# nekStab/nekStab_next

Measured on AMD Instinct MI355X. Metric: Arnoldi-step GB/s (achieved HBM) + Ritz-value rel-err, N=1e8 m=128, higher is better.
Workload: dtype f64

## Files before the change

include/nekkrylov.h:

```cpp
#ifndef NEKKRYLOV_H
#define NEKKRYLOV_H

#include <stddef.h>
#include <stdint.h>

#ifdef __cplusplus
extern "C" {
#endif

#define NKV_ABI_VERSION 3

#define NKV_TILE 4096
#define NKV_MAX_COLS 1024
#define NKV_ROT_MAX_OUT 256

#define NKV_OK 0
#define NKV_EINVAL 1
#define NKV_EHIP 2
#define NKV_ENAN 3
#define NKV_ESHAPE 4
#define NKV_ECALLBACK 5
#define NKV_EBREAKDOWN 6

#define NKV_TIME 0x1u
// ... 38 lines not shown
                 unsigned flags, void* stream);
int nkv_normalize_dev(const nkv_layout* L, double* x, const double* nrm2_dev, double* beta_dev,
                      unsigned flags, void* stream);

int nkv_dot(const nkv_layout* L, const double* w, const double* a, const double* b, double* out_dev,
            void* ws, unsigned flags, void* stream);

int nkv_block_dot(const nkv_layout* L, const double* w, const double* Q, int j, const double* f,
                  double* h_dev, void* ws, unsigned flags, void* stream);
int nkv_block_update(const nkv_layout* L, const double* w, const double* Q, int j, const double* h_dev,
                     double* f, double* nrm2_dev, void* ws, unsigned flags, void* stream);
int nkv_block_update_dot(const nkv_layout* L, const double* w, const double* Q, int j, const double* h_dev,
                         double* f, double* hout_dev, void* ws, unsigned flags, void* stream);
int nkv_arnoldi_finish(const nkv_layout* L, const double* f, const double* nrm2_dev, double* q_out,
                       int j, const double* h1_dev, const double* h2_dev, double* hcol_dev,
                       unsigned flags, void* stream);

int nkv_combine(const nkv_layout* L, const double* Q, int k, const double* y_dev, double* out, unsigned flags,
                void* stream);
int nkv_normalize_store(const nkv_layout* L, const double* f, const double* nrm2_dev, double* q_next,
                        double* beta_dev, unsigned flags, void* stream);
int nkv_mgs2_step(const nkv_layout* L, const double* w, const double* Q, int j, double* f, double* q_out,
                  double* hcol_dev, void* ws, unsigned flags, void* stream);
int nkv_axpy_dot(const nkv_layout* L, const double* w, double* f, const double* alpha_dev, const double* qa,
                 const double* qb, double* out_dev, void* ws, unsigned flags, void* stream);

int nkv_block_dot2(const nkv_layout* L, const double* w, const double* Q, int j, const double* x,
                   const double* y, double* h_dev, void* ws, unsigned flags, void* stream);
int nkv_dcgs2_coef(int m, const double* hq_dev, const double* hw_dev, const double* nrm_prev_dev, double* H_dev,
                   int64_t ldh, double* coef_dev, void* ws, void* stream);
int nkv_dcgs2_update(const nkv_layout* L, const double* w, const double* Q, int m, const double* coef_dev,
                     double* qj, const double* win, double* fout, double* nrm2_dev, void* ws, unsigned flags,
                     void* stream);

int nkv_mgs_icwy_solve(int j, double* G, int64_t ldg, const double* grow, const double* b, double* x,
                       void* stream);

int nkv_gkl_coef(int side, int m, const double* hq_dev, const double* hw_dev, double* M_dev, int64_t ldm,
                 double* A_self, double* r_self, const double* A_other, const double* r_other, int64_t lda,
                 double* coef_dev, void* ws, void* stream);

typedef int (*nkv_matvec_fn)(void* user, const double* x, double* y, void* stream);
typedef int (*nkv_allreduce_fn)(void* user, double* buf, int n, void* stream);
size_t nkv_arnoldi_scratch_doubles(int m);
int nkv_arnoldi_dcgs2(const nkv_layout* L, const double* w, double* Q, int mstart, int mend, double* H_dev,
                      int64_t ldh, double* f, double* scratch_dev, void* ws, nkv_matvec_fn matvec, void* mv_user,
                      nkv_allreduce_fn allreduce, void* ar_user, unsigned flags, void* stream);

int nkv_gmres_dcgs2(const nkv_layout* L, const double* w, double* Q, int kmax, double beta, double tol2,
                    double* H_dev, int64_t ldh, double* f, double* scratch_dev, void* ws, nkv_matvec_fn matvec,
                    void* mv_user, nkv_allreduce_fn allreduce, void* ar_user, double* res_hist, int* k_out,
                    unsigned flags, void* stream);

int nkv_update_hessenberg(const nkv_layout* L, const double* w, const double* Q, int j, double* f, double* q_out,
                          double* hcol_dev, double* scratch_dev, void* ws, nkv_allreduce_fn allreduce, void* ar_user,
                          unsigned flags, void* stream);

int nkv_arnoldi_factorization(const nkv_layout* L, const double* w, double* Q, int mstart, int mend, double* H_dev,
                              int64_t ldh, double* f, double* scratch_dev, void* ws, nkv_matvec_fn matvec,
                              void* mv_user, nkv_allreduce_fn allreduce, void* ar_user, unsigned flags, void* stream);

int nkv_rotate(const nkv_layout* L, double* Q, int k, const double* V_dev, int ldv, void* stream);

int nkv_rotate_cols(const nkv_layout* L, double* Q, int k, const double* V_dev, int ldv, int n_out,
                    void* stream);

// ... 42 lines not shown
```

nekstab_next_amd/_lib.py:

```python
from __future__ import annotations

import ctypes
import os
from ctypes import CFUNCTYPE, POINTER, Structure, c_char_p, c_double, c_int, c_int32, c_int64, c_size_t, c_uint, c_uint64, c_void_p

import torch

_HERE = os.path.dirname(os.path.abspath(__file__))
LIB_PATH = os.path.join(_HERE, "libnekkrylov.so")

NKV_ABI_VERSION = 3
NKV_TILE = 4096
NKV_MAX_COLS = 1024
NKV_ROT_MAX_OUT = 256
NKV_OK, NKV_EINVAL, NKV_EHIP, NKV_ENAN, NKV_ESHAPE, NKV_ECALLBACK, NKV_EBREAKDOWN = 0, 1, 2, 3, 4, 5, 6
NKV_TIME = 0x1
NKV_ACCUMULATE = 0x2
NKV_OVERWRITE = 0x4
NKV_NORM2 = 0x8
NKV_TIME_DOT = 0x10
NKV_X_IS_LAST = 0x20
NKV_MGS2 = 0x40
NKV_MGS_ICWY = 0x100
NKV_MGS_LAGGED = 0x200
# ... 27 lines not shown
        ("n_wf", c_int32),
        ("rank0", c_int32),
    ]


_P = c_void_p
_L = POINTER(nkv_layout)
MATVEC_FN = CFUNCTYPE(c_int, c_void_p, c_void_p, c_void_p, c_void_p)
ALLREDUCE_FN = CFUNCTYPE(c_int, c_void_p, c_void_p, c_int, c_void_p)

_SIGNATURES = {
    "nkv_abi_version": (c_int, []),
    "nkv_layout_init": (c_int, [_L, c_int, c_int, c_int, c_int64, c_int64, c_int, c_int, c_int]),
    "nkv_last_error": (c_char_p, []),
    "nkv_device_info": (c_int, [POINTER(c_int), POINTER(c_int), POINTER(c_int64), c_char_p, c_int]),
    "nkv_workspace_bytes": (c_size_t, [_L, c_int]),
    "nkv_check_status": (c_int, [_P, _P]),
    "nkv_zero": (c_int, [_L, _P, c_uint, _P]),
    "nkv_copy": (c_int, [_L, _P, _P, c_uint, _P]),
    "nkv_scal": (c_int, [_L, _P, c_double, c_uint, _P]),
    "nkv_axpby": (c_int, [_L, _P, c_double, _P, c_double, c_uint, _P]),
    "nkv_sub3": (c_int, [_L, _P, _P, _P, c_uint, _P]),
    "nkv_axpy_dev": (c_int, [_L, _P, _P, c_double, _P, c_uint, _P]),
    "nkv_normalize_dev": (c_int, [_L, _P, _P, _P, c_uint, _P]),
    "nkv_dot": (c_int, [_L, _P, _P, _P, _P, _P, c_uint, _P]),
    "nkv_block_dot": (c_int, [_L, _P, _P, c_int, _P, _P, _P, c_uint, _P]),
    "nkv_block_update": (c_int, [_L, _P, _P, c_int, _P, _P, _P, _P, c_uint, _P]),
    "nkv_block_update_dot": (c_int, [_L, _P, _P, c_int, _P, _P, _P, _P, c_uint, _P]),
    "nkv_arnoldi_finish": (c_int, [_L, _P, _P, _P, c_int, _P, _P, _P, c_uint, _P]),
    "nkv_block_dot2": (c_int, [_L, _P, _P, c_int, _P, _P, _P, _P, c_uint, _P]),
    "nkv_dcgs2_coef": (c_int, [c_int, _P, _P, _P, _P, c_int64, _P, _P, _P]),
    "nkv_mgs_icwy_solve": (c_int, [c_int, _P, c_int64, _P, _P, _P, _P]),
    "nkv_dcgs2_update": (c_int, [_L, _P, _P, c_int, _P, _P, _P, _P, _P, _P, c_uint, _P]),
    "nkv_arnoldi_scratch_doubles": (c_size_t, [c_int]),
    "nkv_arnoldi_dcgs2": (c_int, [_L, _P, _P, c_int, c_int, _P, c_int64, _P, _P, _P, MATVEC_FN, _P, ALLREDUCE_FN, _P,
                                  c_uint, _P]),
    "nkv_update_hessenberg": (c_int, [_L, _P, _P, c_int, _P, _P, _P, _P, _P, ALLREDUCE_FN, _P, c_uint, _P]),
    "nkv_gmres_dcgs2": (c_int, [_L, _P, _P, c_int, c_double, c_double, _P, c_int64, _P, _P, _P, MATVEC_FN, _P,
                                ALLREDUCE_FN, _P, _P, _P, c_uint, _P]),
    "nkv_arnoldi_factorization": (c_int, [_L, _P, _P, c_int, c_int, _P, c_int64, _P, _P, _P, MATVEC_FN, _P,
                                          ALLREDUCE_FN, _P, c_uint, _P]),
    "nkv_combine": (c_int, [_L, _P, c_int, _P, _P, c_uint, _P]),
    "nkv_normalize_store": (c_int, [_L, _P, _P, _P, _P, c_uint, _P]),
    "nkv_mgs2_step": (c_int, [_L, _P, _P, c_int, _P, _P, _P, _P, c_uint, _P]),
    "nkv_axpy_dot": (c_int, [_L, _P, _P, _P, _P, _P, _P, _P, c_uint, _P]),
    "nkv_rotate": (c_int, [_L, _P, c_int, _P, c_int, _P]),
    "nkv_rotate_cols": (c_int, [_L, _P, c_int, _P, c_int, c_int, _P]),
    "nkv_op_diag": (c_int, [_L, _P, _P, _P, c_double, _P]),
    "nkv_op_rot2": (c_int, [_L, _P, _P, _P, _P, _P, c_int, _P]),
    "nkv_op_cdiag": (c_int, [_L, _P, _P, _P, _P, c_int, _P]),
    "nkv_fill_hash": (c_int, [_L, _P, c_uint64, c_int64, c_int64, _P]),
    "nkv_mth_rand_add": (c_int, [_L, c_int, c_int, c_int, c_int64, _P, _P, _P, c_double, c_double, c_double, _P, _P]),
    "nkv_group_average": (c_int, [c_int64, _P, _P, _P, _P]),
    "nkv_symmetric_seed": (c_int, [_L, _P, _P, c_double, _P, _P, _P, _P]),
    "nkv_wavemaker": (c_int, [_L, _P, _P, _P, _P, _P, c_int, _P]),
    "nkv_gradm1": (c_int, [_L, c_int, c_int, _P, _P, _P, _P, _P, c_int, c_int64, _P, c_int64, _P]),
    "nkv_bf_sensitivity": (c_int, [_L, _P, _P, _P, _P, _P, _P, c_int, _P]),
    "nkv_givens_column": (c_double, [c_int, _P, _P, _P, _P]),
    "nkv_lagged_coef": (c_int, [c_int, c_int, _P, _P, c_int64, _P, c_int64, _P]),
    "nkv_gkl_coef": (c_int, [c_int, c_int, _P, _P, _P, c_int64, _P, _P, _P, _P, c_int64, _P, _P, _P]),
    "nkv_sfd_step": (c_int, [_L, _P, _P, _P, _P, _P, _P, _P, _P, c_double, c_double, c_double, c_double, c_double,
                             c_int, _P, _P, c_uint, _P]),
    "nkv_tdf_step": (c_int, [_L, _P, _P, _P, _P, c_double, c_int, _P, _P, c_uint, _P]),
}

EXPORTED = tuple(_SIGNATURES)
# ... 52 lines not shown
```

nekstab_next_amd/arnoldi.py:

```python
from __future__ import annotations

import numpy as np
import torch

from . import _lib
from ._lib import NKV_NORM2, NKV_TIME, NKV_TIME_DOT, NKV_X_IS_LAST
from .operators import LinearOperator
from .vector import Basis, NekContext, NekVector


class HessenbergDev:

    def __init__(self, ctx: NekContext, k: int):
        self.ctx, self.k = ctx, k
        self.t = torch.zeros((k, k + 1), dtype=torch.float64, device=ctx.device)

    def col_ptr(self, c: int) -> int:
        return self.t[c].data_ptr()

    def download(self) -> np.ndarray:
        return np.asfortranarray(self.t.detach().cpu().numpy().T)

    def upload(self, H: np.ndarray) -> None:
        self.t.copy_(torch.as_tensor(np.ascontiguousarray(np.asarray(H, dtype=np.float64).T)).to(self.ctx.device))


def update_hessenberg_matrix(ctx: NekContext, Q: Basis, k: int, f: NekVector, Hd: HessenbergDev,
                             mode: str = "cgs2") -> None:
    j = int(k)
    if j + 1 > Q.k or j > ctx.max_cols:
        raise ValueError(f"step {j} exceeds basis size {Q.k} / max_cols {ctx.max_cols}")
    orthonormalize(ctx, Q, j, f, Q.col_ptr(j), Hd.col_ptr(j - 1), mode)


def orthonormalize(ctx: NekContext, Q: Basis, j: int, f: NekVector, out_ptr: int, hcol_ptr: int,
                   mode: str = "cgs2") -> None:
    w, ws, st = ctx.w.data_ptr(), ctx.ws.data_ptr(), ctx.stream
    if mode == "mgs2-icwy":
        raise ValueError("mode 'mgs2-icwy' keeps the basis's Gram matrix across steps: run it through "
                         "arnoldi_factorization (or use 'mgs2' for a single step)")
    if mode in ("cgs2-native", "mgs2-native"):
        scratch = _native_scratch(ctx, j)
        errors = []
        ar_c = _allreduce_callback(ctx, scratch, errors)
        flags = (NKV_TIME_DOT if ctx.time_in_dot else 0) | (_lib.NKV_MGS2 if mode == "mgs2-native" else 0)
        rc = ctx.lib.nkv_update_hessenberg(ctx._Lp, w, Q.ptr, int(j), f.ptr, out_ptr, hcol_ptr, scratch.data_ptr(), ws,
                                           ar_c, None, flags, st)
        if errors:
            raise errors[0]
        _lib.check(rc, "nkv_update_hessenberg")
        return
    if j == 0:
        tf = NKV_TIME if ctx.time_in_dot else 0
        nrm = ctx.scal[3:4]
        ctx.call("nkv_dot", w, f.ptr, f.ptr, nrm.data_ptr(), ws, tf, st)
        ctx.comm.allreduce_(nrm)
# ... 52 lines not shown
    w, ws, st = ctx.w.data_ptr(), ctx.ws.data_ptr(), ctx.stream
    lay, tm = ctx.layout, ctx.timer
    tf = NKV_TIME if ctx.time_in_dot else 0
    m = j - 1
    h = ctx.hd[: 2 * j]
    hp, cp = h.data_ptr(), ctx.coef.data_ptr()
    u = Q.col_ptr(m)
    if tm:
        tm.begin("block_dot2")
    ctx.call("nkv_block_dot2", w, Q.ptr, j, u, f.ptr, hp, ws, tf | NKV_X_IS_LAST, st)
    if tm:
        tm.end("block_dot2", 8.0 * ((j - 1) * lay.N_w + 2 * lay.N_w + lay.n_v))
    ctx.comm.allreduce_(h)
    nprev = None if first else (nrm2.data_ptr() if nrm2 is not None else hp + 8 * m)
    ctx.call_nl("nkv_dcgs2_coef", m, hp, hp + 8 * j, nprev, Hd.t.data_ptr(), Hd.k + 1, cp, ws, st)
    if tm:
        tm.begin("dcgs2_update")
    ctx.call("nkv_dcgs2_update", w, Q.ptr, m, cp, u, f.ptr, Q.col_ptr(j), None if nrm2 is None else nrm2.data_ptr(),
             ws, NKV_TIME | (NKV_TIME_DOT if tf else 0), st)
    if tm:
        tm.end("dcgs2_update", 8.0 * (m * lay.N + 4 * lay.N) + (0.0 if nrm2 is None else 8.0 * lay.n_v))
    if nrm2 is not None:
        ctx.comm.allreduce_(nrm2)


def _dcgs2_close(ctx: NekContext, Q: Basis, Hd: HessenbergDev, m: int) -> None:
    w, ws, st = ctx.w.data_ptr(), ctx.ws.data_ptr(), ctx.stream
    lay, tm = ctx.layout, ctx.timer
    tf = NKV_TIME if ctx.time_in_dot else 0
    h, coef = ctx.hd[: m + 1], ctx.coef
    u = Q.col_ptr(m)
    if tm:
        tm.begin("block_dot")
    ctx.call("nkv_block_dot", w, Q.ptr, m + 1, u, h.data_ptr(), ws, tf, st)
    if tm:
        tm.end("block_dot", 8.0 * ((m + 1) * lay.N_w + lay.N_w + lay.n_v))
    ctx.comm.allreduce_(h)
    ctx.call_nl("nkv_dcgs2_coef", m, h.data_ptr(), None, h.data_ptr() + 8 * m, Hd.t.data_ptr(), Hd.k + 1,
                coef.data_ptr(), ws, st)
    if tm:
        tm.begin("block_update")
    ctx.call("nkv_block_update", w, Q.ptr, m, h.data_ptr(), u, None, ws, NKV_TIME, st)
    if tm:
        tm.end("block_update", 8.0 * (m * lay.N + 2 * lay.N))
    ctx.call("nkv_normalize_dev", u, coef[2 * m + 3:].data_ptr(), None, 0, st)


def _icwy_gram(ctx: NekContext, Q: Basis, mstart: int) -> torch.Tensor:
    ldg = ctx.max_cols + 1
    G = getattr(ctx, "_icwy_G", None)
    if G is None:
        G = ctx._icwy_G = torch.zeros((ldg, ldg), dtype=torch.float64, device=ctx.device)
    w, ws, st = ctx.w.data_ptr(), ctx.ws.data_ptr(), ctx.stream
    tf = NKV_TIME if ctx.time_in_dot else 0
    for i in range(1, mstart - 1):
        ctx.call("nkv_block_dot", w, Q.ptr, i, Q.col_ptr(i), G[i].data_ptr(), ws, tf, st)
        ctx.comm.allreduce_(G[i, :i])
    return G


def _icwy_step(ctx: NekContext, Q: Basis, Hd: HessenbergDev, j: int, f: NekVector, G: torch.Tensor) -> None:
    w, ws, st = ctx.w.data_ptr(), ctx.ws.data_ptr(), ctx.stream
    lay, tm = ctx.layout, ctx.timer
    tf = NKV_TIME if ctx.time_in_dot else 0
    ldg = G.shape[1]
    h = ctx.hd[: 2 * j]
    hp, gp = h.data_ptr(), G.data_ptr()
    h1, h2, nrm = ctx.h1[:j], ctx.h2[:j], ctx.scal[3:4]
    if tm:
        tm.begin("block_dot2")
    ctx.call("nkv_block_dot2", w, Q.ptr, j, Q.col_ptr(j - 1), f.ptr, hp, ws, tf | NKV_X_IS_LAST, st)
    if tm:
        tm.end("block_dot2", 8.0 * ((j - 1) * lay.N_w + 2 * lay.N_w + lay.n_v))
    ctx.comm.allreduce_(h)
    ctx.call_nl("nkv_mgs_icwy_solve", j, gp, ldg, hp, hp + 8 * j, h1.data_ptr(), st)
    b_upd = 8.0 * (j * lay.N + 2 * lay.N)
    if tm:
        tm.begin("update_dot")
# ... 133 lines not shown
    scratch = _native_scratch(ctx, mend)
    base, ld8, fptr = Q.ptr, 8 * ctx.layout.ld, f.ptr
    apply = op.rmatvec if transpose else op.matvec
    errors = []

    def matvec(_user, x, y, _stream):
        try:
            c, r = divmod((x or 0) - base, ld8)
            if r or not 0 <= c < Q.k or y != fptr:
                raise ValueError(f"{entry} matvec callback: x={x}, y={y} are not a basis column and f")
            apply(Q[c], f)
            return 0
        except BaseException as e:
            errors.append(e)
            return 1

    mv_c = _lib.MATVEC_FN(matvec)
    ar_c = _allreduce_callback(ctx, scratch, errors)
    rc = getattr(lib, entry)(ctx._Lp, ctx.w.data_ptr(), Q.ptr, int(mstart), int(mend), Hd.t.data_ptr(), Hd.k + 1,
                             fptr, scratch.data_ptr(), ctx.ws.data_ptr(), mv_c, None, ar_c, None,
                             (NKV_TIME_DOT if ctx.time_in_dot else 0) | flags, ctx.stream)
    if errors:
        raise errors[0]
    _lib.check(rc, entry)


def arnoldi_factorization(ctx: NekContext, op: LinearOperator, Q: Basis, Hd: HessenbergDev, mstart: int,
                          mend: int, f: NekVector | None = None, mode: str = "cgs2", transpose: bool = False,
                          on_step=None) -> None:
    if mend < mstart:
        return
    if Q.k < mend + 1:
        raise ValueError("basis too small")
    if f is None:
        f = ctx.vector()
    if mode == "dcgs2-native":
        if on_step is None:
            if mend > ctx.max_cols or mend + 1 > Hd.k + 1:
                raise ValueError(f"step {mend} exceeds max_cols {ctx.max_cols} / H size {Hd.k}")
            _dcgs2_native(ctx, op, Q, Hd, mstart, mend, f, transpose)
            return
        mode = "dcgs2"
    if mode == "dcgs2" and on_step is not None:
        if mend > ctx.max_cols or mend + 1 > Hd.k + 1:
            raise ValueError(f"step {mend} exceeds max_cols {ctx.max_cols} / H size {Hd.k}")
        for mstep in range(mstart, mend + 1):
            (op.rmatvec if transpose else op.matvec)(Q[mstep - 1], f)
            _dcgs2_step(ctx, Q, Hd, mstep, f, first=(mstep == mstart))
            if mstep > mstart:
                on_step(mstep - 1)
        _dcgs2_close(ctx, Q, Hd, mend)
        on_step(mend)
        return
    if mode == "mgs2-lagged-native":
        if on_step is None:
            if mend > ctx.max_cols or mend + 1 > Hd.k + 1:
                raise ValueError(f"step {mend} exceeds max_cols {ctx.max_cols} / H size {Hd.k}")
            _dcgs2_native(ctx, op, Q, Hd, mstart, mend, f, transpose, entry="nkv_arnoldi_factorization",
                          flags=_lib.NKV_MGS_LAGGED)
            return
        mode = "mgs2-lagged"
    if mode == "mgs2-lagged":
        if mend > ctx.max_cols or mend + 1 > Hd.k + 1:
            raise ValueError(f"step {mend} exceeds max_cols {ctx.max_cols} / H size {Hd.k}")
        _lagged_factorization(ctx, op, Q, Hd, mstart, mend, f, transpose, on_step)
        return
# ... 26 lines not shown
            raise ValueError(f"step {mend} exceeds max_cols {ctx.max_cols} / H size {Hd.k}")
        for mstep in range(mstart, mend + 1):
            (op.rmatvec if transpose else op.matvec)(Q[mstep - 1], f)
            _dcgs2_step(ctx, Q, Hd, mstep, f, first=(mstep == mstart))
        _dcgs2_close(ctx, Q, Hd, mend)
        return
    if mode == "dcgs2":
        mode = "cgs2"
    for mstep in range(mstart, mend + 1):
        x = Q[mstep - 1]
        (op.rmatvec if transpose else op.matvec)(x, f)
        update_hessenberg_matrix(ctx, Q, mstep, f, Hd, mode)
        if on_step is not None:
            on_step(mstep)


class FactorizationGraph:

    def __init__(self, ctx: NekContext, op: LinearOperator, Q: Basis, Hd: HessenbergDev, f: NekVector,
                 mode: str = "cgs2"):
        self.ctx, self.op, self.Q, self.Hd, self.f, self.mode = ctx, op, Q, Hd, f, mode
        self.graphs = {}

    HOST_SYNC_MODES = ("mgs2-lagged", "mgs2-lagged-native")

    def usable(self) -> bool:
        return self.ctx.comm.world == 1 and self.mode not in self.HOST_SYNC_MODES

    def run(self, mstart: int, mend: int, transpose: bool = False) -> None:
        if mend < mstart:
            return
        key = (mstart, mend, transpose)
        Q = self.Q
        g = self.graphs.get(key)
        if g is None:
            timer, self.ctx.timer = self.ctx.timer, None
            g = torch.cuda.CUDAGraph()
            torch.cuda.synchronize(self.ctx.device)
            with torch.cuda.graph(g):
                arnoldi_factorization(self.ctx, self.op, Q, self.Hd, mstart, mend, f=self.f, mode=self.mode,
                                      transpose=transpose)
            self.ctx.timer = timer
            self.graphs[key] = g
        g.replay()
```

nekstab_next_amd/csrc/drivers.hip:

```cpp
#include "nkv_internal.h"

#include <vector>

extern "C" {

static size_t icwy_scratch_doubles(int m) { return (size_t)(4 * (m + 1) + 2) + (size_t)(m + 1) * (size_t)(m + 1); }
size_t nkv_arnoldi_scratch_doubles(int m) {
    const size_t base = (size_t)(2 * (m + 1) + 4 * m + 16), icwy = icwy_scratch_doubles(m);
    return base > icwy ? base : icwy;
}

static constexpr double kBreakdownTol = 1e-8;

static int check_breakdown(const double* H_dev, int64_t ldh, int c0, int c1, void* ws, void* stream) {
    if (c0 < 0) c0 = 0;
    if (c1 <= c0) return NKV_OK;
    hipStream_t st = S(stream);
    const size_t n = (size_t)ldh * (size_t)(c1 - c0);
    double* h = static_cast<double*>(malloc(n * sizeof(double)));
    if (!h) return fail(NKV_EINVAL, "breakdown check: host allocation of %zu doubles failed", n);
    int flag = 0;
    hipError_t e = hipMemcpyAsync(h, H_dev + (int64_t)c0 * ldh, n * sizeof(double), hipMemcpyDeviceToHost, st);
    if (e == hipSuccess) e = hipMemcpyAsync(&flag, nan_flag_of(ws), sizeof(int), hipMemcpyDeviceToHost, st);
    if (e == hipSuccess) e = hipStreamSynchronize(st);
// ... 20 lines not shown
        return fail(NKV_EBREAKDOWN, "breakdown at column %d: |H(c+1,c)|/||H(:,c)|| = %.3g (invariant subspace)",
                    bad, ratio);
    return NKV_OK;
}

int nkv_arnoldi_dcgs2(const nkv_layout* L, const double* w, double* Q, int mstart, int mend, double* H_dev,
                      int64_t ldh, double* f, double* scratch_dev, void* ws, nkv_matvec_fn matvec, void* mv_user,
                      nkv_allreduce_fn allreduce, void* ar_user, unsigned flags, void* stream) {
    CHECK(check_layout(L));
    CHECK(check_ptr(Q, "Q"));
    CHECK(check_ptr(f, "f"));
    if (!matvec) return fail(NKV_EINVAL, "matvec callback is NULL");
    if (!H_dev || !scratch_dev) return fail(NKV_EINVAL, "H/scratch is NULL");
    if (mstart < 1 || mend > NKV_MAX_COLS) return fail(NKV_EINVAL, "steps %d..%d outside 1..%d", mstart, mend, NKV_MAX_COLS);
    if (mend < mstart) return NKV_OK;
    if (ldh < mend + 1) return fail(NKV_EINVAL, "ldh=%lld < mend+1=%d", (long long)ldh, mend + 1);
    const unsigned tf = (flags & NKV_TIME_DOT) ? NKV_TIME : 0u;
    double* hd = scratch_dev;
    double* coef = scratch_dev + 2 * (mend + 1);
    auto col = [L, Q](int c) { return Q + (int64_t)c * L->ld; };
    for (int j = mstart; j <= mend; ++j) {
        const int m = j - 1;
        double* u = col(m);
        int rc = matvec(mv_user, u, f, stream);
        if (rc != 0) return fail(NKV_ECALLBACK, "matvec callback returned %d at step %d", rc, j);
        CHECK(nkv_block_dot2(L, w, Q, j, u, f, hd, ws, tf | NKV_X_IS_LAST, stream));
        if (allreduce && (rc = allreduce(ar_user, hd, 2 * j, stream)) != 0)
            return fail(NKV_ECALLBACK, "allreduce callback returned %d at step %d", rc, j);
        CHECK(nkv_dcgs2_coef(m, hd, hd + j, j == mstart ? nullptr : hd + m, H_dev, ldh, coef, ws, stream));
        CHECK(nkv_dcgs2_update(L, w, Q, m, coef, u, f, col(j), nullptr, ws, NKV_TIME, stream));
    }
    const int m = mend;
    double* u = col(m);
    CHECK(nkv_block_dot(L, w, Q, m + 1, u, hd, ws, tf, stream));
    if (allreduce) {
        const int rc = allreduce(ar_user, hd, m + 1, stream);
        if (rc != 0) return fail(NKV_ECALLBACK, "allreduce callback returned %d (closing step)", rc);
    }
    CHECK(nkv_dcgs2_coef(m, hd, nullptr, hd + m, H_dev, ldh, coef, ws, stream));
    CHECK(nkv_block_update(L, w, Q, m, hd, u, nullptr, ws, NKV_TIME, stream));
    CHECK(nkv_normalize_dev(L, u, coef + 2 * m + 3, nullptr, 0, stream));
    return (flags & NKV_CHECK_BREAKDOWN) ? check_breakdown(H_dev, ldh, mstart - 1, mend, ws, stream) : NKV_OK;
}

int nkv_gmres_dcgs2(const nkv_layout* L, const double* w, double* Q, int kmax, double beta, double tol2,
                    double* H_dev, int64_t ldh, double* f, double* scratch_dev, void* ws, nkv_matvec_fn matvec,
                    void* mv_user, nkv_allreduce_fn allreduce, void* ar_user, double* res_hist, int* k_out,
                    unsigned flags, void* stream) {
    CHECK(check_layout(L));
    CHECK(check_ptr(Q, "Q"));
    CHECK(check_ptr(f, "f"));
    CHECK(check_ptr(w, "w"));
    CHECK(check_ptr(ws, "ws"));
    if (!matvec) return fail(NKV_EINVAL, "matvec callback is NULL");
    if (!H_dev || !scratch_dev || !res_hist || !k_out) return fail(NKV_EINVAL, "H/scratch/res_hist/k_out is NULL");
    if (kmax < 1 || kmax + 1 > NKV_MAX_COLS) return fail(NKV_EINVAL, "kmax=%d outside 1..%d", kmax, NKV_MAX_COLS - 1);
    if (ldh < kmax + 1) return fail(NKV_EINVAL, "ldh=%lld < kmax+1=%d", (long long)ldh, kmax + 1);
    hipStream_t st = S(stream);
    const unsigned tf = (flags & NKV_TIME_DOT) ? NKV_TIME : 0u;
    double* hd = scratch_dev;
    double* coef = scratch_dev + 2 * (kmax + 1);
    double* nrm2 = scratch_dev + nkv_arnoldi_scratch_doubles(kmax) - 1;
    double* host = nullptr;
    if (hipHostMalloc(reinterpret_cast<void**>(&host), sizeof(double) * (size_t)(4 * (kmax + 2)),
                      hipHostMallocDefault) != hipSuccess || !host)
        return fail(NKV_EHIP, "gmres: pinned host allocation failed");
    double *h = host, *cs = host + (kmax + 2), *sn = cs + (kmax + 2), *g = sn + (kmax + 2);
    for (int i = 0; i < kmax + 2; ++i) g[i] = 0.0;
    g[0] = beta;
    auto col = [L, Q](int c) { return Q + (int64_t)c * L->ld; };
    auto reduce = [&](double* buf, int n, const char* what) -> int {
        if (!allreduce) return NKV_OK;
        const int rc = allreduce(ar_user, buf, n, stream);
        return rc == 0 ? NKV_OK : fail(NKV_ECALLBACK, "allreduce callback returned %d (%s)", rc, what);
// ... 307 lines not shown
```

nekstab_next_amd/csrc/gram_schmidt.hip:

```cpp
#include "nkv_internal.h"

namespace {

template <bool OVERWRITE, bool NORM, int kPairs>
__global__ __launch_bounds__(kThreads) void k_block_update(const double* __restrict__ Q, int64_t ld,
                                                           int j, const double* __restrict__ h,
                                                           double* __restrict__ f,
                                                           const double* __restrict__ w, int64_t sv,
                                                           int tiles_per_field, int tiles_w,
                                                           int tiles_total, int64_t time_off,
                                                           int do_time,
                                                           double* __restrict__ partials, int t_lo,
                                                           int acc_part) {
    constexpr int kTile = kThreads * kPairs * 2;
    __shared__ double lds4[4];
    if (do_time && blockIdx.x == 0 && threadIdx.x < 64) {
        double s = 0.0;
        for (int c = threadIdx.x; c < j; c += 64) s = fma(Q[time_off + (int64_t)c * ld], h[c], s);
        s = wave_sum(s);
        if (threadIdx.x == 0) f[time_off] = OVERWRITE ? s : f[time_off] - s;
    }
    double nrm = 0.0;
    for (int t = t_lo + blockIdx.x; t < tiles_total; t += gridDim.x) {
        const int64_t r0 = (int64_t)t * kTile + 2 * threadIdx.x;
// ... 545 lines not shown
int launch_block_update_p(const nkv_layout* L, const double* w, const double* Q, int j, const double* h_dev,
                          double* f, double* part, unsigned flags, hipStream_t st, int* g_out) {
    constexpr int kTile = kThreads * P * 2;
    const bool over = (flags & NKV_OVERWRITE) != 0;
    const bool norm = (flags & NKV_NORM2) != 0;
    const int tpf = (int)(L->sv / kTile);
    const int tiles_w = tpf * L->n_wf;
    const int tiles_total = (int)(rows_of(L) / kTile);
    const int gmax = j <= NKV_UPD_SMALL_J ? 4 * kMaxBlocks : kMaxBlocks;
    int g = tiles_total < gmax ? tiles_total : gmax;
    if (g < 1) g = 1;
    *g_out = g;
    const int64_t T = rows_of(L);
    const int dt = (flags & NKV_TIME) ? 1 : 0;
    auto kern = over ? (norm ? k_block_update<true, true, P> : k_block_update<true, false, P>)
                     : (norm ? k_block_update<false, true, P> : k_block_update<false, false, P>);
    const int64_t b = (int64_t)NKV_UPD_ROUNDS * g;
    const int band = (NKV_UPD_ROUNDS <= 0 || b >= tiles_total || tiles_total < 2 * b) ? (tiles_total > 0 ? tiles_total : 1)
                                                                                        : (int)b;
    for (int lo = 0; lo == 0 || lo < tiles_total; lo += band) {
        const int hi = lo + band < tiles_total ? lo + band : tiles_total;
        const int gb = lo == 0 ? g : (g < hi - lo ? g : hi - lo);
        hipLaunchKernelGGL(kern, dim3(gb), dim3(kThreads), 0, st, Q, L->ld, j, h_dev, f, w, L->sv, tpf, tiles_w, hi, T,
                           lo == 0 ? dt : 0, part, lo, lo == 0 ? 0 : 1);
        NKV_LAUNCHED();
    }
    return NKV_OK;
}

inline int band_tiles(int tiles_total, int g) {
    if (NKV_DC_ROUNDS <= 0) return tiles_total > 0 ? tiles_total : 1;
    const int64_t b = (int64_t)NKV_DC_ROUNDS * g;
    return (b >= tiles_total || tiles_total < 2 * b) ? (tiles_total > 0 ? tiles_total : 1) : (int)b;
}

__global__ __launch_bounds__(kThreads) void k_mgs_icwy_solve(int j, double* __restrict__ G, int64_t ldg,
                                                             const double* __restrict__ grow,
                                                             const double* b, double* x) {
    extern __shared__ double xs[];
    for (int i = threadIdx.x; i < j; i += kThreads) xs[i] = b[i];
    if (grow)
        for (int k = threadIdx.x; k < j - 1; k += kThreads) G[(int64_t)(j - 1) * ldg + k] = grow[k];
    for (int k = 0; k + 1 < j; ++k) {
        __syncthreads();
        const double xk = xs[k];
        for (int i = k + 1 + threadIdx.x; i < j; i += kThreads) {
            const double g = (grow && i == j - 1) ? grow[k] : G[(int64_t)i * ldg + k];
            xs[i] = xs[i] - g * xk;
        }
    }
    __syncthreads();
    for (int i = threadIdx.x; i < j; i += kThreads) x[i] = xs[i];
}

}

extern "C" {

int nkv_block_update(const nkv_layout* L, const double* w, const double* Q, int j, const double* h_dev,
                     double* f, double* nrm2_dev, void* ws, unsigned flags, void* stream) {
    CHECK(check_layout(L));
    CHECK(check_ptr(Q, "Q"));
    CHECK(check_ptr(f, "f"));
    if (!h_dev) return fail(NKV_EINVAL, "h_dev is NULL");
    if (j < 0) return fail(NKV_EINVAL, "j=%d < 0", j);
    const bool norm = (flags & NKV_NORM2) != 0;
// ... 196 lines not shown
    const bool large = use_large_tiles(L);
    const int P = large ? NKV_DC_PAIRS : NKV_PAIRS_SMALL;
    const int kTile = kThreads * P * 2;
    const int tpf = (int)(L->sv / kTile);
    const int tiles_w = tpf * L->n_wf;
    const int tiles_total = (int)(rows_of(L) / kTile);
    const int gmax = NKV_DC_G < kMaxBlocks ? NKV_DC_G : kMaxBlocks;
    int g = tiles_total < gmax ? tiles_total : gmax;
    if (g < 1) g = 1;
    const int64_t T = rows_of(L);
    const int dt = (flags & NKV_TIME) ? 1 : 0;
    double* part = partials_of(ws);
    auto kern = large ? (nrm2_dev ? k_dcgs2_update<NKV_DC_PAIRS, true> : k_dcgs2_update<NKV_DC_PAIRS, false>)
                      : (nrm2_dev ? k_dcgs2_update<NKV_PAIRS_SMALL, true> : k_dcgs2_update<NKV_PAIRS_SMALL, false>);
    if (!nrm2_dev) {
        const int band = band_tiles(tiles_total, g);
        for (int lo = 0; lo == 0 || lo < tiles_total; lo += band) {
            const int hi = lo + band < tiles_total ? lo + band : tiles_total;
            const int gb = g < hi - lo ? g : (hi - lo > 0 ? hi - lo : 1);
            hipLaunchKernelGGL(kern, dim3(gb), dim3(kThreads), 0, st, Q, L->ld, m, coef_dev, qj, win, fout, w, L->sv,
                               tpf, tiles_w, tiles_total, T, lo == 0 ? dt : 0, part, lo, hi);
            NKV_LAUNCHED();
        }
        return NKV_OK;
    }
    hipLaunchKernelGGL(kern, dim3(g), dim3(kThreads), 0, st, Q, L->ld, m, coef_dev, qj, win, fout, w, L->sv, tpf,
                       tiles_w, tiles_total, T, dt, part, 0, tiles_total);
    NKV_LAUNCHED();
    const bool tdot = (flags & NKV_TIME_DOT) && L->rank0;
    CHECK(launch_reduce_cols(1, part, g, nrm2_dev, tdot ? fout + T : nullptr, (int64_t)0, tdot ? fout + T : nullptr, nullptr, 1 << 30, nan_flag_of(ws), st));
    return NKV_OK;
}

int nkv_combine(const nkv_layout* L, const double* Q, int k, const double* y_dev, double* out, unsigned flags,
                void* stream) {
    return nkv_block_update(L, nullptr, Q, k, y_dev, out, nullptr, nullptr,
                            (flags & ~(unsigned)NKV_NORM2) | NKV_OVERWRITE, stream);
}

}
```

nekstab_next_amd/csrc/vector.hip:

```cpp
#include "nkv_internal.h"

namespace {

template <int kPairs>
__global__ __launch_bounds__(kThreads) void k_block_dot(const double* __restrict__ Q, int64_t ld,
                                                        int j, const double* __restrict__ f,
                                                        const double* __restrict__ w, int64_t sv,
                                                        int tiles_per_field,
                                                        double* __restrict__ partials, int B) {
    constexpr int kTile = kThreads * kPairs * 2;
    extern __shared__ double red[];
    const int wave = threadIdx.x >> 6, lane = threadIdx.x & 63;
    for (int c = threadIdx.x; c < 4 * j; c += kThreads) red[c] = 0.0;
    __syncthreads();

    const int64_t fb = (int64_t)blockIdx.y * sv;
    for (int t = blockIdx.x; t < tiles_per_field; t += gridDim.x) {
        const int64_t r0 = (int64_t)t * kTile + 2 * threadIdx.x;
        double2 wf[kPairs];
#pragma unroll
        for (int k = 0; k < kPairs; ++k) {
            const double2 wv = ld2(w + r0 + k * 2 * kThreads);
            const double2 fv = ld2(f + fb + r0 + k * 2 * kThreads);
            wf[k].x = wv.x * fv.x;
            wf[k].y = wv.y * fv.y;
        }
        const double* qb = Q + fb + r0;
        int c = 0;
        for (; c + kColUnroll <= j; c += kColUnroll) {
            double2 q[kColUnroll][kPairs];
#pragma unroll
            for (int u = 0; u < kColUnroll; ++u)
#pragma unroll
                for (int k = 0; k < kPairs; ++k) q[u][k] = ldq(qb + (int64_t)(c + u) * ld + k * 2 * kThreads);
            double s[kColUnroll];
#pragma unroll
            for (int u = 0; u < kColUnroll; ++u) {
                double a = 0.0;
#pragma unroll
                for (int k = 0; k < kPairs; ++k) {
                    a = fma(q[u][k].x, wf[k].x, a);
                    a = fma(q[u][k].y, wf[k].y, a);
                }
                s[u] = a;
            }
#if NKV_D2_RED && NKV_COLU == 4
            const double v = wave_sum4(s[0], s[1], s[2], s[3], lane);
            if ((lane & 15) == 0) red[wave * j + c + (lane >> 4)] += v;
#else
#pragma unroll
            for (int off = 32; off > 0; off >>= 1)
#pragma unroll
                for (int u = 0; u < kColUnroll; ++u) s[u] += __shfl_xor(s[u], off, 64);
            if (lane == 0) {
#pragma unroll
                for (int u = 0; u < kColUnroll; ++u) red[wave * j + c + u] += s[u];
            }
#endif
        }
        for (; c < j; ++c) {
            double a = 0.0;
#pragma unroll
            for (int k = 0; k < kPairs; ++k) {
                const double2 q = ldq(qb + (int64_t)c * ld + k * 2 * kThreads);
                a = fma(q.x, wf[k].x, a);
                a = fma(q.y, wf[k].y, a);
            }
            a = wave_sum(a);
            if (lane == 0) red[wave * j + c] += a;
        }
    }
    __syncthreads();
    const int b = blockIdx.y * gridDim.x + blockIdx.x;
    for (int c = threadIdx.x; c < j; c += kThreads)
        partials[(int64_t)c * B + b] = (red[c] + red[j + c]) + (red[2 * j + c] + red[3 * j + c]);
}

__global__ __launch_bounds__(kThreads) void k_reduce_cols(const double* __restrict__ partials, int B,
                                                          double* __restrict__ out,
                                                          const double* __restrict__ ta, int64_t lda,
                                                          const double* __restrict__ tb,
                                                          const double* __restrict__ tb2, int jc,
                                                          int* __restrict__ nan_flag) {
    __shared__ double lds4[4];
    const int c = blockIdx.x;
    double s = 0.0;
    for (int b = threadIdx.x; b < B; b += kThreads) s += partials[(int64_t)c * B + b];
    s = block_sum(s, lds4);
    if (threadIdx.x == 0) {
        if (ta) s += (c < jc) ? ta[(int64_t)c * lda] * tb[0] : ta[(int64_t)(c - jc) * lda] * tb2[0];
        if (s != s) atomicOr(nan_flag, 1);
        out[c] = s;
    }
}

template <int kPairs>
__global__ __launch_bounds__(kThreads) void k_axpy_dot(const double* __restrict__ qa,
                                                       const double* __restrict__ alpha,
                                                       double* __restrict__ f,
                                                       const double* __restrict__ qb,
                                                       const double* __restrict__ w, int64_t sv,
                                                       int tiles_per_field, int tiles_w, int tiles_total,
// ... 93 lines not shown
                r = make_double2(xv[u].x * a + yv[u].x * b, xv[u].y * a + yv[u].y * b);
            if (OP == OP_SUB3) r = make_double2(yv[u].x - zv[u].x, yv[u].y - zv[u].y);
            if (OP == OP_AXPY_DEV) r = make_double2(fma(a, yv[u].x, xv[u].x), fma(a, yv[u].y, xv[u].y));
            st2(x + 2 * (p0 + u * kThreads), r);
        }
    }
    if (do_time && blockIdx.x == 0 && threadIdx.x == 0) {
        const int64_t i = time_off;
        if (OP == OP_ZERO) x[i] = 0.0;
        if (OP == OP_COPY) x[i] = y[i];
        if (OP == OP_SCAL) x[i] = x[i] * a;
        if (OP == OP_AXPBY) x[i] = x[i] * a + y[i] * b;
        if (OP == OP_SUB3) x[i] = y[i] - z[i];
        if (OP == OP_AXPY_DEV) x[i] = fma(a, y[i], x[i]);
    }
}

__global__ void k_accumulate(double* __restrict__ dst, const double* __restrict__ src) {
    if (threadIdx.x == 0) dst[0] += src[0];
}

template <int P>
int launch_block_dot_p(const nkv_layout* L, const double* w, const double* Q, int64_t ld, int j,
                       const double* f, double* out, void* ws, unsigned flags, hipStream_t st) {
    constexpr int kTile = kThreads * P * 2;
    const int tpf = (int)(L->sv / kTile);
    const int bmax = (P == NKV_PAIRS_SMALL && P != NKV_PAIRS && NKV_DOT_SMALL_B < kMaxBlocks) ? NKV_DOT_SMALL_B : kMaxBlocks;
    int bx = bmax / L->n_wf;
    if (bx > tpf) bx = tpf;
    if (bx < 1) bx = 1;
    const int B = bx * L->n_wf;
    double* part = partials_of(ws);
    if (tpf > 0) {
        hipLaunchKernelGGL(k_block_dot<P>, dim3(bx, L->n_wf), dim3(kThreads), 4 * j * sizeof(double), st,
                           Q, ld, j, f, w, L->sv, tpf, part, B);
        NKV_LAUNCHED();
    }
    const int64_t T = rows_of(L);
    const bool tdot = (flags & NKV_TIME) && L->rank0;
    hipLaunchKernelGGL(k_reduce_cols, dim3(j), dim3(kThreads), 0, st, part, tpf > 0 ? B : 0, out,
                       tdot ? Q + T : nullptr, ld, tdot ? f + T : nullptr, nullptr, 1 << 30, nan_flag_of(ws));
    NKV_LAUNCHED();
    return NKV_OK;
}

}

namespace nkvi {

int launch_block_dot(const nkv_layout* L, const double* w, const double* Q, int64_t ld, int j,
                     const double* f, double* out, void* ws, unsigned flags, hipStream_t st) {
    return use_large_tiles(L) ? launch_block_dot_p<NKV_PAIRS>(L, w, Q, ld, j, f, out, ws, flags, st)
                              : launch_block_dot_p<NKV_PAIRS_SMALL>(L, w, Q, ld, j, f, out, ws, flags, st);
}

int launch_reduce_cols(int ncols, const double* partials, int B, double* out, const double* ta, int64_t lda,
                       const double* tb, const double* tb2, int jc, int* nan_flag, hipStream_t st) {
    hipLaunchKernelGGL(k_reduce_cols, dim3(ncols), dim3(kThreads), 0, st, partials, B, out, ta, lda, tb, tb2, jc,
                       nan_flag);
    NKV_LAUNCHED();
    return NKV_OK;
}

}

extern "C" {

// ... 37 lines not shown
             void* stream) {
    CHECK(check_ptr(q, "q"));
    CHECK(check_ptr(r, "r"));
    return blas1(L, OP_SUB3, p, q, r, 0, 0, nullptr, flags, stream);
}
int nkv_axpy_dev(const nkv_layout* L, double* x, const double* alpha_dev, double sign,
                 const double* y, unsigned flags, void* stream) {
    CHECK(check_ptr(y, "y"));
    if (!alpha_dev) return fail(NKV_EINVAL, "alpha_dev is NULL");
    return blas1(L, OP_AXPY_DEV, x, y, nullptr, 0, sign, alpha_dev, flags, stream);
}

int nkv_normalize_dev(const nkv_layout* L, double* x, const double* nrm2_dev, double* beta_dev,
                      unsigned flags, void* stream) {
    (void)flags;
    CHECK(check_layout(L));
    CHECK(check_ptr(x, "x"));
    if (!nrm2_dev) return fail(NKV_EINVAL, "nrm2_dev is NULL");
    const int64_t rows = rows_of(L);
    hipLaunchKernelGGL(k_finish, dim3(grid_for(rows / 2)), dim3(kThreads), 0, S(stream), x, nrm2_dev,
                       x, rows, rows, 0, nullptr, nullptr, nullptr, beta_dev);
    NKV_LAUNCHED();
    return NKV_OK;
}

int nkv_dot(const nkv_layout* L, const double* w, const double* a, const double* b, double* out_dev,
            void* ws, unsigned flags, void* stream) {
    CHECK(check_layout(L));
    CHECK(check_ptr(w, "w"));
    CHECK(check_ptr(a, "a"));
    CHECK(check_ptr(b, "b"));
    CHECK(check_ptr(ws, "ws"));
    if (!out_dev) return fail(NKV_EINVAL, "out_dev is NULL");
    return launch_block_dot(L, w, a, L->ld, 1, b, out_dev, ws, flags, S(stream));
}

int nkv_block_dot(const nkv_layout* L, const double* w, const double* Q, int j, const double* f,
                  double* h_dev, void* ws, unsigned flags, void* stream) {
    CHECK(check_layout(L));
    CHECK(check_ptr(w, "w"));
    CHECK(check_ptr(Q, "Q"));
    CHECK(check_ptr(f, "f"));
    CHECK(check_ptr(ws, "ws"));
    if (!h_dev) return fail(NKV_EINVAL, "h_dev is NULL");
    if (j < 1 || j > NKV_MAX_COLS) return fail(NKV_EINVAL, "j=%d outside 1..%d", j, NKV_MAX_COLS);
    return launch_block_dot(L, w, Q, L->ld, j, f, h_dev, ws, flags, S(stream));
}

int nkv_arnoldi_finish(const nkv_layout* L, const double* f, const double* nrm2_dev, double* q_out,
                       int j, const double* h1_dev, const double* h2_dev, double* hcol_dev,
                       unsigned flags, void* stream) {
    (void)flags;
    CHECK(check_layout(L));
    CHECK(check_ptr(f, "f"));
    CHECK(check_ptr(q_out, "q_out"));
    if (!nrm2_dev) return fail(NKV_EINVAL, "nrm2_dev is NULL");
    if (hcol_dev && (!h1_dev || j < 0)) return fail(NKV_EINVAL, "hcol needs h1 and j >= 0");
    const int64_t rows = rows_of(L);
    hipLaunchKernelGGL(k_finish, dim3(grid_for(rows / 2)), dim3(kThreads), 0, S(stream), f, nrm2_dev,
                       q_out, rows, rows, j, h1_dev, h2_dev, hcol_dev, nullptr);
    NKV_LAUNCHED();
    return NKV_OK;
}

int nkv_normalize_store(const nkv_layout* L, const double* f, const double* nrm2_dev, double* q_next,
                        double* beta_dev, unsigned flags, void* stream) {
    (void)flags;
    CHECK(check_layout(L));
    CHECK(check_ptr(f, "f"));
    CHECK(check_ptr(q_next, "q_next"));
    if (!nrm2_dev) return fail(NKV_EINVAL, "nrm2_dev is NULL");
    const int64_t rows = rows_of(L);
    hipLaunchKernelGGL(k_finish, dim3(grid_for(rows / 2)), dim3(kThreads), 0, S(stream), f, nrm2_dev, q_next, rows,
                       rows, 0, nullptr, nullptr, nullptr, beta_dev);
    NKV_LAUNCHED();
    return NKV_OK;
}

// ... 77 lines not shown
```

Baseline: 6886.

## Fuse DCGS2 closing update with normalization and skip redundant self-column read

The closing step of the DCGS2 Arnoldi factorization now uses a new fused kernel that subtracts the projection and applies the normalization in one pass over u, replacing separate block_update and normalize_dev passes. The block dot gains an X_IS_LAST mode that computes the self inner product from the already loaded f values instead of reading the last Q column a second time. Downloading H after a final mark now goes through a pinned-host async copy on a side stream. Together these cut HBM traffic and launch overhead on the closing step, at the cost of an extra kernel variant and new event bookkeeping.

```diff
diff --git a/include/nekkrylov.h b/include/nekkrylov.h
--- a/include/nekkrylov.h
+++ b/include/nekkrylov.h
@@ -94,6 +94,8 @@
 int nkv_dcgs2_update(const nkv_layout* L, const double* w, const double* Q, int m, const double* coef_dev,
                      double* qj, const double* win, double* fout, double* nrm2_dev, void* ws, unsigned flags,
                      void* stream);
+int nkv_dcgs2_close(const nkv_layout* L, const double* Q, int m, const double* h_dev, const double* nrm2_dev,
+                    double* u, unsigned flags, void* stream);
 
 int nkv_mgs_icwy_solve(int j, double* G, int64_t ldg, const double* grow, const double* b, double* x,
                        void* stream);
diff --git a/nekstab_next_amd/_lib.py b/nekstab_next_amd/_lib.py
--- a/nekstab_next_amd/_lib.py
+++ b/nekstab_next_amd/_lib.py
@@ -83,6 +83,7 @@
     "nkv_dcgs2_coef": (c_int, [c_int, _P, _P, _P, _P, c_int64, _P, _P, _P]),
     "nkv_mgs_icwy_solve": (c_int, [c_int, _P, c_int64, _P, _P, _P, _P]),
     "nkv_dcgs2_update": (c_int, [_L, _P, _P, c_int, _P, _P, _P, _P, _P, _P, c_uint, _P]),
+    "nkv_dcgs2_close": (c_int, [_L, _P, c_int, _P, _P, _P, c_uint, _P]),
     "nkv_arnoldi_scratch_doubles": (c_size_t, [c_int]),
     "nkv_arnoldi_dcgs2": (c_int, [_L, _P, _P, c_int, c_int, _P, c_int64, _P, _P, _P, MATVEC_FN, _P, ALLREDUCE_FN, _P,
                                   c_uint, _P]),
diff --git a/nekstab_next_amd/arnoldi.py b/nekstab_next_amd/arnoldi.py
--- a/nekstab_next_amd/arnoldi.py
+++ b/nekstab_next_amd/arnoldi.py
@@ -14,14 +14,39 @@
     def __init__(self, ctx: NekContext, k: int):
         self.ctx, self.k = ctx, k
         self.t = torch.zeros((k, k + 1), dtype=torch.float64, device=ctx.device)
+        self._final = None
+        self._side = None
+        self._host = None
 
     def col_ptr(self, c: int) -> int:
         return self.t[c].data_ptr()
 
+    def mark_final(self) -> None:
+        if torch.cuda.is_current_stream_capturing():
+            self._final = None
+            return
+        ev = torch.cuda.Event()
+        ev.record(torch.cuda.current_stream(self.ctx.device))
+        self._final = ev
+
+    def invalidate(self) -> None:
+        self._final = None
+
     def download(self) -> np.ndarray:
-        return np.asfortranarray(self.t.detach().cpu().numpy().T)
+        ev, self._final = self._final, None
+        if ev is None:
+            return np.asfortranarray(self.t.detach().cpu().numpy().T)
+        if self._side is None:
+            self._side = torch.cuda.Stream(self.ctx.device)
+            self._host = torch.empty((self.k, self.k + 1), dtype=torch.float64, pin_memory=True)
+        self._side.wait_event(ev)
+        with torch.cuda.stream(self._side):
+            self._host.copy_(self.t, non_blocking=True)
+        self._side.synchronize()
+        return self._host.numpy().T.copy(order="F")
 
     def upload(self, H: np.ndarray) -> None:
+        self._final = None
         self.t.copy_(torch.as_tensor(np.ascontiguousarray(np.asarray(H, dtype=np.float64).T)).to(self.ctx.device))
 
 
@@ -140,18 +165,18 @@
     u = Q.col_ptr(m)
     if tm:
         tm.begin("block_dot")
-    ctx.call("nkv_block_dot", w, Q.ptr, m + 1, u, h.data_ptr(), ws, tf, st)
-    if tm:
-        tm.end("block_dot", 8.0 * ((m + 1) * lay.N_w + lay.N_w + lay.n_v))
+    ctx.call("nkv_block_dot", w, Q.ptr, m + 1, u, h.data_ptr(), ws, tf | NKV_X_IS_LAST, st)
+    if tm:
+        tm.end("block_dot", 8.0 * (m * lay.N_w + lay.N_w + lay.n_v))
     ctx.comm.allreduce_(h)
     ctx.call_nl("nkv_dcgs2_coef", m, h.data_ptr(), None, h.data_ptr() + 8 * m, Hd.t.data_ptr(), Hd.k + 1,
                 coef.data_ptr(), ws, st)
+    Hd.mark_final()
     if tm:
         tm.begin("block_update")
-    ctx.call("nkv_block_update", w, Q.ptr, m, h.data_ptr(), u, None, ws, NKV_TIME, st)
+    ctx.call("nkv_dcgs2_close", Q.ptr, m, h.data_ptr(), coef.data_ptr() + 8 * (2 * m + 3), u, NKV_TIME, st)
     if tm:
         tm.end("block_update", 8.0 * (m * lay.N + 2 * lay.N))
-    ctx.call("nkv_normalize_dev", u, coef[2 * m + 3:].data_ptr(), None, 0, st)
 
 
 def _icwy_gram(ctx: NekContext, Q: Basis, mstart: int) -> torch.Tensor:
@@ -351,6 +376,7 @@
         return
     if Q.k < mend + 1:
         raise ValueError("basis too small")
+    Hd._final = None
     if f is None:
         f = ctx.vector()
     if mode == "dcgs2-native":
@@ -443,6 +469,7 @@
             return
         key = (mstart, mend, transpose)
         Q = self.Q
+        self.Hd._final = None
         g = self.graphs.get(key)
         if g is None:
             timer, self.ctx.timer = self.ctx.timer, None
diff --git a/nekstab_next_amd/csrc/drivers.hip b/nekstab_next_amd/csrc/drivers.hip
--- a/nekstab_next_amd/csrc/drivers.hip
+++ b/nekstab_next_amd/csrc/drivers.hip
@@ -76,14 +76,13 @@
     }
     const int m = mend;
     double* u = col(m);
-    CHECK(nkv_block_dot(L, w, Q, m + 1, u, hd, ws, tf, stream));
+    CHECK(nkv_block_dot(L, w, Q, m + 1, u, hd, ws, tf | NKV_X_IS_LAST, stream));
     if (allreduce) {
         const int rc = allreduce(ar_user, hd, m + 1, stream);
         if (rc != 0) return fail(NKV_ECALLBACK, "allreduce callback returned %d (closing step)", rc);
     }
     CHECK(nkv_dcgs2_coef(m, hd, nullptr, hd + m, H_dev, ldh, coef, ws, stream));
-    CHECK(nkv_block_update(L, w, Q, m, hd, u, nullptr, ws, NKV_TIME, stream));
-    CHECK(nkv_normalize_dev(L, u, coef + 2 * m + 3, nullptr, 0, stream));
+    CHECK(nkv_dcgs2_close(L, Q, m, hd, coef + 2 * m + 3, u, NKV_TIME, stream));
     return (flags & NKV_CHECK_BREAKDOWN) ? check_breakdown(H_dev, ldh, mstart - 1, mend, ws, stream) : NKV_OK;
 }
 
diff --git a/nekstab_next_amd/csrc/gram_schmidt.hip b/nekstab_next_amd/csrc/gram_schmidt.hip
--- a/nekstab_next_amd/csrc/gram_schmidt.hip
+++ b/nekstab_next_amd/csrc/gram_schmidt.hip
@@ -601,6 +601,63 @@
     if (NKV_DC_ROUNDS <= 0) return tiles_total > 0 ? tiles_total : 1;
     const int64_t b = (int64_t)NKV_DC_ROUNDS * g;
     return (b >= tiles_total || tiles_total < 2 * b) ? (tiles_total > 0 ? tiles_total : 1) : (int)b;
+}
+
+template <int kPairs>
+__global__ __launch_bounds__(kThreads)
+void k_dcgs2_close(const double* __restrict__ Q, int64_t ld, int m, const double* __restrict__ h,
+                   const double* __restrict__ nrm2, double* __restrict__ u, int64_t time_off, int do_scalar,
+                   int do_time, int t_lo, int t_hi) {
+    constexpr int kTile = kThreads * kPairs * 2;
+    const double beta = sqrt(nrm2[0]);
+    const double inv = 1.0 / beta;
+    if (do_scalar && blockIdx.x == 0 && threadIdx.x < 64) {
+        double s = 0.0;
+        if (do_time) {
+            for (int c = threadIdx.x; c < m; c += 64) s = fma(Q[time_off + (int64_t)c * ld], h[c], s);
+            s = wave_sum(s);
+        }
+        if (threadIdx.x == 0) {
+            const double ut = do_time ? u[time_off] - s : u[time_off];
+            u[time_off] = ut * inv;
+        }
+    }
+    constexpr int U = NKV_DC_U;
+    for (int t = t_lo + blockIdx.x; t < t_hi; t += gridDim.x) {
+        const int64_t r0 = (int64_t)t * kTile + 2 * threadIdx.x;
+        double2 acc[kPairs];
+#pragma unroll
+        for (int k = 0; k < kPairs; ++k) acc[k] = ld2(u + r0 + k * 2 * kThreads);
+        const double* qb = Q + r0;
+        int c = 0;
+        for (; c + U <= m; c += U) {
+            double2 q[U][kPairs];
+#pragma unroll
+            for (int v = 0; v < U; ++v)
+#pragma unroll
+                for (int k = 0; k < kPairs; ++k) q[v][k] = ldq(qb + (int64_t)(c + v) * ld + k * 2 * kThreads);
+#pragma unroll
+            for (int v = 0; v < U; ++v) {
+                const double hc = -h[c + v];
+#pragma unroll
+                for (int k = 0; k < kPairs; ++k) {
+                    acc[k].x = fma(hc, q[v][k].x, acc[k].x);
+                    acc[k].y = fma(hc, q[v][k].y, acc[k].y);
+                }
+            }
+        }
+        for (; c < m; ++c) {
+            const double hc = -h[c];
+#pragma unroll
+            for (int k = 0; k < kPairs; ++k) {
+                const double2 q = ldq(qb + (int64_t)c * ld + k * 2 * kThreads);
+                acc[k].x = fma(hc, q.x, acc[k].x);
+                acc[k].y = fma(hc, q.y, acc[k].y);
+            }
+        }
+#pragma unroll
+        for (int k = 0; k < kPairs; ++k) st2p(u, r0 + k * 2 * kThreads, make_double2(acc[k].x * inv, acc[k].y * inv));
+    }
 }
 
 __global__ __launch_bounds__(kThreads) void k_mgs_icwy_solve(int j, double* __restrict__ G, int64_t ldg,
@@ -863,6 +920,34 @@
     return NKV_OK;
 }
 
+int nkv_dcgs2_close(const nkv_layout* L, const double* Q, int m, const double* h_dev, const double* nrm2_dev,
+                    double* u, unsigned flags, void* stream) {
+    CHECK(check_layout(L));
+    CHECK(check_ptr(u, "u"));
+    if (m < 0) return fail(NKV_EINVAL, "m=%d < 0", m);
+    if (m > 0) CHECK(check_ptr(Q, "Q"));
+    if (!h_dev || !nrm2_dev) return fail(NKV_EINVAL, "h_dev/nrm2_dev is NULL");
+    hipStream_t st = S(stream);
+    const bool large = use_large_tiles(L);
+    const int kTile = kThreads * (large ? NKV_DC_PAIRS : NKV_PAIRS_SMALL) * 2;
+    const int tiles_total = (int)(rows_of(L) / kTile);
+    const int gmax = NKV_DC_G < kMaxBlocks ? NKV_DC_G : kMaxBlocks;
+    int g = tiles_total < gmax ? tiles_total : gmax;
+    if (g < 1) g = 1;
+    const int64_t T = rows_of(L);
+    const int dt = (flags & NKV_TIME) ? 1 : 0;
+    auto kern = large ? k_dcgs2_close<NKV_DC_PAIRS> : k_dcgs2_close<NKV_PAIRS_SMALL>;
+    const int band = band_tiles(tiles_total, g);
+    for (int lo = 0; lo == 0 || lo < tiles_total; lo += band) {
+        const int hi = lo + band < tiles_total ? lo + band : tiles_total;
+        const int gb = g < hi - lo ? g : (hi - lo > 0 ? hi - lo : 1);
+        hipLaunchKernelGGL(kern, dim3(gb), dim3(kThreads), 0, st, Q, L->ld, m, h_dev, nrm2_dev, u, T, lo == 0 ? 1 : 0,
+                           dt, lo, hi);
+        NKV_LAUNCHED();
+    }
+    return NKV_OK;
+}
+
 int nkv_combine(const nkv_layout* L, const double* Q, int k, const double* y_dev, double* out, unsigned flags,
                 void* stream) {
     return nkv_block_update(L, nullptr, Q, k, y_dev, out, nullptr, nullptr,
diff --git a/nekstab_next_amd/csrc/vector.hip b/nekstab_next_amd/csrc/vector.hip
--- a/nekstab_next_amd/csrc/vector.hip
+++ b/nekstab_next_amd/csrc/vector.hip
@@ -2,7 +2,7 @@
 
 namespace {
 
-template <int kPairs>
+template <int kPairs, bool XL>
 __global__ __launch_bounds__(kThreads) void k_block_dot(const double* __restrict__ Q, int64_t ld,
                                                         int j, const double* __restrict__ f,
                                                         const double* __restrict__ w, int64_t sv,
@@ -14,20 +14,27 @@
     for (int c = threadIdx.x; c < 4 * j; c += kThreads) red[c] = 0.0;
     __syncthreads();
 
+    const int jl = XL ? j - 1 : j;
+    const bool tree4 = XL && NKV_D2_RED && kColUnroll == 4 && j % kColUnroll == 0;
     const int64_t fb = (int64_t)blockIdx.y * sv;
     for (int t = blockIdx.x; t < tiles_per_field; t += gridDim.x) {
         const int64_t r0 = (int64_t)t * kTile + 2 * threadIdx.x;
         double2 wf[kPairs];
+        double sff = 0.0;
 #pragma unroll
         for (int k = 0; k < kPairs; ++k) {
             const double2 wv = ld2(w + r0 + k * 2 * kThreads);
             const double2 fv = ld2(f + fb + r0 + k * 2 * kThreads);
             wf[k].x = wv.x * fv.x;
             wf[k].y = wv.y * fv.y;
+            if (XL) {
+                sff = fma(fv.x, wf[k].x, sff);
+                sff = fma(fv.y, wf[k].y, sff);
+            }
         }
         const double* qb = Q + fb + r0;
         int c = 0;
-        for (; c + kColUnroll <= j; c += kColUnroll) {
+        for (; c + kColUnroll <= jl; c += kColUnroll) {
             double2 q[kColUnroll][kPairs];
 #pragma unroll
             for (int u = 0; u < kColUnroll; ++u)
@@ -58,7 +65,7 @@
             }
 #endif
         }
-        for (; c < j; ++c) {
+        for (; c < jl; ++c) {
             double a = 0.0;
 #pragma unroll
             for (int k = 0; k < kPairs; ++k) {
@@ -66,8 +73,12 @@
                 a = fma(q.x, wf[k].x, a);
                 a = fma(q.y, wf[k].y, a);
             }
-            a = wave_sum(a);
+            a = tree4 ? wave_sum4(a, a, a, a, lane) : wave_sum(a);
             if (lane == 0) red[wave * j + c] += a;
+        }
+        if (XL) {
+            const double a = tree4 ? wave_sum4(sff, sff, sff, sff, lane) : wave_sum(sff);
+            if (lane == 0) red[wave * j + j - 1] += a;
         }
     }
     __syncthreads();
@@ -227,7 +238,8 @@
     const int B = bx * L->n_wf;
     double* part = partials_of(ws);
     if (tpf > 0) {
-        hipLaunchKernelGGL(k_block_dot<P>, dim3(bx, L->n_wf), dim3(kThreads), 4 * j * sizeof(double), st,
+        auto kern = (flags & NKV_X_IS_LAST) ? k_block_dot<P, true> : k_block_dot<P, false>;
+        hipLaunchKernelGGL(kern, dim3(bx, L->n_wf), dim3(kThreads), 4 * j * sizeof(double), st,
                            Q, ld, j, f, w, L->sv, tpf, part, B);
         NKV_LAUNCHED();
     }
@@ -331,7 +343,7 @@
     CHECK(check_ptr(b, "b"));
     CHECK(check_ptr(ws, "ws"));
     if (!out_dev) return fail(NKV_EINVAL, "out_dev is NULL");
-    return launch_block_dot(L, w, a, L->ld, 1, b, out_dev, ws, flags, S(stream));
+    return launch_block_dot(L, w, a, L->ld, 1, b, out_dev, ws, flags & ~(unsigned)NKV_X_IS_LAST, S(stream));
 }
 
 int nkv_block_dot(const nkv_layout* L, const double* w, const double* Q, int j, const double* f,
@@ -343,6 +355,8 @@
     CHECK(check_ptr(ws, "ws"));
     if (!h_dev) return fail(NKV_EINVAL, "h_dev is NULL");
     if (j < 1 || j > NKV_MAX_COLS) return fail(NKV_EINVAL, "j=%d outside 1..%d", j, NKV_MAX_COLS);
+    if ((flags & NKV_X_IS_LAST) && f != Q + (int64_t)(j - 1) * L->ld)
+        return fail(NKV_EINVAL, "NKV_X_IS_LAST: f is not column j-1 of Q");
     return launch_block_dot(L, w, Q, L->ld, j, f, h_dev, ws, flags, S(stream));
 }
 
```

After: 6914, median of 6. No clear change (+0.4%).
